# 0xk0ry/HTR-VT

Measured on NVIDIA B200. Metric: line images/sec (train step), higher is better.
Workload: dtype bf16

## Files before the change

### htr-vt_b200/csrc/attention.cu

```cuda
#include "common.cuh"
#include <cuda.h>

namespace htrvt {

constexpr int kAttnThreads = 160;
constexpr int kHd = 128;
constexpr int kTq = 128;
constexpr int kImg = kTq * 128;

__device__ __forceinline__ uint64_t desc_kmajor(uint32_t img, int k16) {
  return umma_desc_sw128(img + (k16 >> 2) * kImg + (k16 & 3) * 32, 16, 1024);
}
__device__ __forceinline__ uint64_t desc_mnmajor(uint32_t img, int k16) {
  return umma_desc_sw128(img + k16 * 2048, kImg, 1024);
}
__device__ __forceinline__ void img_store8(uint8_t* img, int r, int c, int g, uint4 v) {
  *reinterpret_cast<uint4*>(img + c * kImg + r * 128 + ((g ^ (r & 7)) << 4)) = v;
}

__device__ __forceinline__ void load_image(uint8_t* dst, const CUtensorMap* map, uint64_t* bar, int col0, int row0,
                                           int z) {
  tma_load_3d(dst, map, bar, col0, row0, z);
  tma_load_3d(dst + kImg, map, bar, col0 + 64, row0, z);
}

struct AttnP {
  int B, H, T;
  float scale;
  __nv_bfloat16* out;
  float* lse;
  const __nv_bfloat16* o;
  const __nv_bfloat16* dout;
  __nv_bfloat16* dqkv;
};

__global__ void __launch_bounds__(kAttnThreads, 2)
attn_fwd_kernel(const __grid_constant__ CUtensorMap tmQKV, const __grid_constant__ AttnP P) {
  extern __shared__ uint8_t smem_raw[];
  uint8_t* smem = reinterpret_cast<uint8_t*>((reinterpret_cast<uintptr_t>(smem_raw) + 1023) & ~uintptr_t(1023));
  uint8_t* sQ = smem;
  uint8_t* sK = smem + 2 * kImg;
  uint8_t* sV = smem + 4 * kImg;
  uint8_t* sP = sQ;
  uint64_t* bars = reinterpret_cast<uint64_t*>(smem + 6 * kImg);
  uint64_t* bar_load = bars, *bar_s = bars + 1, *bar_p = bars + 2, *bar_o = bars + 3;
  uint32_t* tmem_slot = reinterpret_cast<uint32_t*>(bars + 4);

  const int warp = threadIdx.x >> 5, lane = threadIdx.x & 31;
  const int bh = blockIdx.x, b = bh / P.H, h = bh - b * P.H;

  if (warp == 4 && lane == 0) {
    tma_prefetch_desc(&tmQKV);
    mbar_init(bar_load, 1); mbar_init(bar_s, 1); mbar_init(bar_p, 128); mbar_init(bar_o, 1);
    fence_barrier_init();
  }
  if (warp == 4) tmem_alloc(tmem_slot, 256);
  tc_fence_before();
  __syncthreads();
  tc_fence_after();
  const uint32_t tmem = *tmem_slot;
  constexpr uint32_t idesc_s = umma_idesc_bf16(128, 128, 0, 0);
  constexpr uint32_t idesc_o = umma_idesc_bf16(128, 128, 0, 1);

  if (warp == 4) {
    if (lane == 0) {
      mbar_arrive_expect_tx(bar_load, 6 * kImg);
      const int D = P.H * kHd;
      load_image(sQ, &tmQKV, bar_load, h * kHd, 0, b);
      load_image(sK, &tmQKV, bar_load, D + h * kHd, 0, b);
      load_image(sV, &tmQKV, bar_load, 2 * D + h * kHd, 0, b);
      mbar_wait(bar_load, 0);
      tc_fence_after();
      const uint32_t q = smem_u32(sQ), k = smem_u32(sK);
#pragma unroll
      for (int i = 0; i < 8; ++i) umma_bf16(tmem, desc_kmajor(q, i), desc_kmajor(k, i), idesc_s, i ? 1u : 0u);
      umma_commit(bar_s);
      mbar_wait(bar_p, 0);
      tc_fence_after();
      const uint32_t pp = smem_u32(sP), v = smem_u32(sV);
#pragma unroll
      for (int i = 0; i < 8; ++i) umma_bf16(tmem + 128, desc_kmajor(pp, i), desc_mnmajor(v, i), idesc_o, i ? 1u : 0u);
      umma_commit(bar_o);
    }
  } else {
    const int r = warp * 32 + lane;
    const uint32_t trow = tmem + (static_cast<uint32_t>(warp * 32) << 16);
    mbar_wait(bar_s, 0);
    tc_fence_after();
    float s[128];
#pragma unroll
    for (int c = 0; c < 128; c += 16) {
      uint32_t raw[16];
      tmem_ld16(trow + c, raw);
      tmem_ld_wait();
#pragma unroll
      for (int i = 0; i < 16; ++i) s[c + i] = __uint_as_float(raw[i]);
    }
    const float sl2 = P.scale * kLog2e;
    float m = -INFINITY;
#pragma unroll
    for (int j = 0; j < 128; ++j) {
      if (j >= P.T) s[j] = -INFINITY;
      m = fmaxf(m, s[j]);
    }
    float sum = 0.f;
#pragma unroll
    for (int j = 0; j < 128; ++j) {
      s[j] = ex2f((s[j] - m) * sl2);
      sum += s[j];
    }
    const float inv = __fdividef(1.0f, sum);
    asm volatile("bar.sync 1, 128;" ::: "memory");
#pragma unroll
    for (int g = 0; g < 16; ++g) {
      uint4 u;
      u.x = pack_bf16(s[8 * g], s[8 * g + 1]); u.y = pack_bf16(s[8 * g + 2], s[8 * g + 3]);
      u.z = pack_bf16(s[8 * g + 4], s[8 * g + 5]); u.w = pack_bf16(s[8 * g + 6], s[8 * g + 7]);
      img_store8(sP, r, g >> 3, g & 7, u);
    }
    fence_proxy_async();
    tc_fence_before();
    mbar_arrive(bar_p);
    if (r < P.T && P.lse) P.lse[static_cast<long long>(bh) * P.T + r] = m * P.scale + __logf(sum);
    mbar_wait(bar_o, 0);
    tc_fence_after();
    __nv_bfloat16* orow = P.out + (static_cast<long long>(b) * P.T + r) * (P.H * kHd) + h * kHd;
#pragma unroll
    for (int c = 0; c < 128; c += 16) {
      uint32_t raw[16];
      tmem_ld16(trow + 128 + c, raw);
      tmem_ld_wait();
      if (r < P.T) {
        uint4 u0, u1;
        u0.x = pack_bf16(__uint_as_float(raw[0]) * inv, __uint_as_float(raw[1]) * inv);
        u0.y = pack_bf16(__uint_as_float(raw[2]) * inv, __uint_as_float(raw[3]) * inv);
        u0.z = pack_bf16(__uint_as_float(raw[4]) * inv, __uint_as_float(raw[5]) * inv);
        u0.w = pack_bf16(__uint_as_float(raw[6]) * inv, __uint_as_float(raw[7]) * inv);
        u1.x = pack_bf16(__uint_as_float(raw[8]) * inv, __uint_as_float(raw[9]) * inv);
        u1.y = pack_bf16(__uint_as_float(raw[10]) * inv, __uint_as_float(raw[11]) * inv);
        u1.z = pack_bf16(__uint_as_float(raw[12]) * inv, __uint_as_float(raw[13]) * inv);
        u1.w = pack_bf16(__uint_as_float(raw[14]) * inv, __uint_as_float(raw[15]) * inv);
        *reinterpret_cast<uint4*>(orow + c) = u0;
        *reinterpret_cast<uint4*>(orow + c + 8) = u1;
      }
    }
  }
  tc_fence_before();
  __syncthreads();
  if (warp == 4) tmem_dealloc(tmem, 256);
}

__global__ void __launch_bounds__(kAttnThreads, 1)
attn_bwd_kernel(const __grid_constant__ CUtensorMap tmQKV, const __grid_constant__ CUtensorMap tmDO,
                const __grid_constant__ AttnP P) {
  extern __shared__ uint8_t smem_raw[];
  uint8_t* smem = reinterpret_cast<uint8_t*>((reinterpret_cast<uintptr_t>(smem_raw) + 1023) & ~uintptr_t(1023));
  uint8_t* sQ = smem;
  uint8_t* sK = smem + 2 * kImg;
  uint8_t* sV = smem + 4 * kImg;
  uint8_t* sDO = smem + 6 * kImg;
  uint8_t* sP = smem + 8 * kImg;
  uint8_t* sDS = smem + 10 * kImg;
  uint64_t* bars = reinterpret_cast<uint64_t*>(smem + 12 * kImg);
  uint64_t* bar_load = bars, *bar_s = bars + 1, *bar_p = bars + 2, *bar_g = bars + 3;
  uint32_t* tmem_slot = reinterpret_cast<uint32_t*>(bars + 4);

  const int warp = threadIdx.x >> 5, lane = threadIdx.x & 31;
  const int bh = blockIdx.x, b = bh / P.H, h = bh - b * P.H;

  if (warp == 4 && lane == 0) {
    tma_prefetch_desc(&tmQKV);
    tma_prefetch_desc(&tmDO);
    mbar_init(bar_load, 1); mbar_init(bar_s, 1); mbar_init(bar_p, 128); mbar_init(bar_g, 1);
    fence_barrier_init();
  }
  if (warp == 4) tmem_alloc(tmem_slot, 512);
  tc_fence_before();
  __syncthreads();
  tc_fence_after();
  const uint32_t tmem = *tmem_slot;
  constexpr uint32_t id_kk = umma_idesc_bf16(128, 128, 0, 0);
  constexpr uint32_t id_km = umma_idesc_bf16(128, 128, 0, 1);
  constexpr uint32_t id_mm = umma_idesc_bf16(128, 128, 1, 1);

  if (warp == 4) {
    if (lane == 0) {
      mbar_arrive_expect_tx(bar_load, 8 * kImg);
      const int Dm = P.H * kHd;
      load_image(sQ, &tmQKV, bar_load, h * kHd, 0, b);
      load_image(sK, &tmQKV, bar_load, Dm + h * kHd, 0, b);
      load_image(sV, &tmQKV, bar_load, 2 * Dm + h * kHd, 0, b);
      load_image(sDO, &tmDO, bar_load, h * kHd, 0, b);
      mbar_wait(bar_load, 0);
      tc_fence_after();
      const uint32_t q = smem_u32(sQ), k = smem_u32(sK), v = smem_u32(sV), d_o = smem_u32(sDO);
      const uint32_t pp = smem_u32(sP), ds = smem_u32(sDS);
#pragma unroll
      for (int i = 0; i < 8; ++i) umma_bf16(tmem, desc_kmajor(q, i), desc_kmajor(k, i), id_kk, i ? 1u : 0u);
#pragma unroll
      for (int i = 0; i < 8; ++i) umma_bf16(tmem + 128, desc_kmajor(d_o, i), desc_kmajor(v, i), id_kk, i ? 1u : 0u);
      umma_commit(bar_s);
      mbar_wait(bar_p, 0);
      tc_fence_after();
#pragma unroll
      for (int i = 0; i < 8; ++i) umma_bf16(tmem + 384, desc_mnmajor(pp, i), desc_mnmajor(d_o, i), id_mm, i ? 1u : 0u);
#pragma unroll
      for (int i = 0; i < 8; ++i) umma_bf16(tmem, desc_mnmajor(ds, i), desc_mnmajor(q, i), id_mm, i ? 1u : 0u);
#pragma unroll
      for (int i = 0; i < 8; ++i) umma_bf16(tmem + 256, desc_kmajor(ds, i), desc_mnmajor(k, i), id_km, i ? 1u : 0u);
      umma_commit(bar_g);
    }
  } else {
    const int r = warp * 32 + lane;
    const bool rok = r < P.T;
    const uint32_t trow = tmem + (static_cast<uint32_t>(warp * 32) << 16);
    const int D = P.H * kHd;
    float delta = 0.f;
    if (rok) {
      const uint4* po = reinterpret_cast<const uint4*>(P.o + (static_cast<long long>(b) * P.T + r) * D + h * kHd);
      const uint4* pd = reinterpret_cast<const uint4*>(P.dout + (static_cast<long long>(b) * P.T + r) * D + h * kHd);
#pragma unroll 4
      for (int i = 0; i < 16; ++i) {
        const uint4 a = __ldg(po + i), c = __ldg(pd + i);
        float2 x, y;
        x = unpack_bf16(a.x); y = unpack_bf16(c.x); delta += x.x * y.x + x.y * y.y;
        x = unpack_bf16(a.y); y = unpack_bf16(c.y); delta += x.x * y.x + x.y * y.y;
        x = unpack_bf16(a.z); y = unpack_bf16(c.z); delta += x.x * y.x + x.y * y.y;
        x = unpack_bf16(a.w); y = unpack_bf16(c.w); delta += x.x * y.x + x.y * y.y;
      }
    }
    const float lse = rok ? P.lse[static_cast<long long>(bh) * P.T + r] : 0.f;
    mbar_wait(bar_s, 0);
    tc_fence_after();
    const float sl2 = P.scale * kLog2e, lse2 = lse * kLog2e;
#pragma unroll 1
    for (int c = 0; c < 128; c += 16) {
      uint32_t rs[16], rp[16];
      tmem_ld16(trow + c, rs);
      tmem_ld16(trow + 128 + c, rp);
      tmem_ld_wait();
      float p[16], ds[16];
#pragma unroll
      for (int i = 0; i < 16; ++i) {
        const bool ok = rok && (c + i) < P.T;
        p[i] = ok ? ex2f(__uint_as_float(rs[i]) * sl2 - lse2) : 0.f;
        ds[i] = ok ? p[i] * (__uint_as_float(rp[i]) - delta) * P.scale : 0.f;
      }
#pragma unroll
      for (int g = 0; g < 2; ++g) {
        uint4 u, w;
        u.x = pack_bf16(p[8 * g], p[8 * g + 1]); u.y = pack_bf16(p[8 * g + 2], p[8 * g + 3]);
        u.z = pack_bf16(p[8 * g + 4], p[8 * g + 5]); u.w = pack_bf16(p[8 * g + 6], p[8 * g + 7]);
        w.x = pack_bf16(ds[8 * g], ds[8 * g + 1]); w.y = pack_bf16(ds[8 * g + 2], ds[8 * g + 3]);
        w.z = pack_bf16(ds[8 * g + 4], ds[8 * g + 5]); w.w = pack_bf16(ds[8 * g + 6], ds[8 * g + 7]);
        const int gg = (c >> 3) + g;
        img_store8(sP, r, gg >> 3, gg & 7, u);
        img_store8(sDS, r, gg >> 3, gg & 7, w);
      }
    }
    fence_proxy_async();
    tc_fence_before();
    mbar_arrive(bar_p);
    mbar_wait(bar_g, 0);
    tc_fence_after();
    __nv_bfloat16* base = P.dqkv + (static_cast<long long>(b) * P.T + r) * (3 * D) + h * kHd;
    const uint32_t cols[3] = {256u, 0u, 384u};
#pragma unroll 1
    for (int w = 0; w < 3; ++w) {
      __nv_bfloat16* dst = base + w * D;
#pragma unroll 1
      for (int c = 0; c < 128; c += 16) {
        uint32_t raw[16];
        tmem_ld16(trow + cols[w] + c, raw);
        tmem_ld_wait();
        if (rok) {
          uint4 u0, u1;
          u0.x = pack_bf16(__uint_as_float(raw[0]), __uint_as_float(raw[1]));
          u0.y = pack_bf16(__uint_as_float(raw[2]), __uint_as_float(raw[3]));
          u0.z = pack_bf16(__uint_as_float(raw[4]), __uint_as_float(raw[5]));
          u0.w = pack_bf16(__uint_as_float(raw[6]), __uint_as_float(raw[7]));
          u1.x = pack_bf16(__uint_as_float(raw[8]), __uint_as_float(raw[9]));
          u1.y = pack_bf16(__uint_as_float(raw[10]), __uint_as_float(raw[11]));
          u1.z = pack_bf16(__uint_as_float(raw[12]), __uint_as_float(raw[13]));
          u1.w = pack_bf16(__uint_as_float(raw[14]), __uint_as_float(raw[15]));
          *reinterpret_cast<uint4*>(dst + c) = u0;
          *reinterpret_cast<uint4*>(dst + c + 8) = u1;
        }
      }
    }
  }
  tc_fence_before();
  __syncthreads();
  if (warp == 4) tmem_dealloc(tmem, 512);
}

}

using namespace htrvt;

namespace {
typedef CUresult (*EncodeTiledFn)(CUtensorMap*, CUtensorMapDataType, cuuint32_t, void*, const cuuint64_t*,
                                  const cuuint64_t*, const cuuint32_t*, const cuuint32_t*, CUtensorMapInterleave,
                                  CUtensorMapSwizzle, CUtensorMapL2promotion, CUtensorMapFloatOOBfill);
EncodeTiledFn attn_encode() {
  static EncodeTiledFn fn = nullptr;
  if (!fn) {
    void* p = nullptr;
    cudaDriverEntryPointQueryResult q;
    if (cudaGetDriverEntryPoint("cuTensorMapEncodeTiled", &p, cudaEnableDefault, &q) == cudaSuccess &&
        q == cudaDriverEntryPointSuccess)
      fn = reinterpret_cast<EncodeTiledFn>(p);
  }
  return fn;
}
int map3(CUtensorMap* m, const void* ptr, long long cols, long long rows, long long z, long long row_stride,
         long long z_stride) {
  EncodeTiledFn enc = attn_encode();
  if (!enc) return HTRVT_ERR_DRIVER;
  if (reinterpret_cast<uintptr_t>(ptr) & 15) return HTRVT_ERR_ALIGN;
  cuuint64_t gd[3] = {static_cast<cuuint64_t>(cols), static_cast<cuuint64_t>(rows), static_cast<cuuint64_t>(z)};
  cuuint64_t gs[2] = {static_cast<cuuint64_t>(row_stride) * 2, static_cast<cuuint64_t>(z_stride) * 2};
  cuuint32_t bx[3] = {64, 128, 1}, es[3] = {1, 1, 1};
  if ((gs[0] & 15) || (gs[1] & 15)) return HTRVT_ERR_ALIGN;
  CUresult r = enc(m, CU_TENSOR_MAP_DATA_TYPE_BFLOAT16, 3, const_cast<void*>(ptr), gd, gs, bx, es,
                   CU_TENSOR_MAP_INTERLEAVE_NONE, CU_TENSOR_MAP_SWIZZLE_128B, CU_TENSOR_MAP_L2_PROMOTION_L2_256B,
                   CU_TENSOR_MAP_FLOAT_OOB_FILL_NONE);
  return r == CUDA_SUCCESS ? HTRVT_OK : HTRVT_ERR_DRIVER;
}
}

extern "C" int htrvt_attention_fwd(const void* qkv, int B, int H, int T, int hd, float scale, void* out, float* lse,
                                   cudaStream_t stream) {
  if (hd != kHd || T < 1 || T > kTq || B < 1 || H < 1) return HTRVT_ERR_SHAPE;
  CUtensorMap tm;
  int r = map3(&tm, qkv, 3LL * H * kHd, T, B, 3LL * H * kHd, static_cast<long long>(T) * 3 * H * kHd);
  if (r) return r;
  AttnP P = {};
  P.B = B; P.H = H; P.T = T; P.scale = scale; P.out = static_cast<__nv_bfloat16*>(out); P.lse = lse;
  const int smem = 6 * kImg + 1024 + 128;
  if (!HTRVT_ENSURE_SMEM(attn_fwd_kernel, smem)) return HTRVT_ERR_LAUNCH;
  attn_fwd_kernel<<<B * H, kAttnThreads, smem, stream>>>(tm, P);
  HTRVT_LAUNCH_CHECK();
  return HTRVT_OK;
}

extern "C" int htrvt_attention_bwd(const void* qkv, const void* out, const void* dout, const float* lse, int B, int H,
                                   int T, int hd, float scale, void* dqkv, cudaStream_t stream) {
  if (hd != kHd || T < 1 || T > kTq || B < 1 || H < 1 || !lse) return HTRVT_ERR_SHAPE;
  CUtensorMap tm, tdo;
  int r = map3(&tm, qkv, 3LL * H * kHd, T, B, 3LL * H * kHd, static_cast<long long>(T) * 3 * H * kHd);
  if (r) return r;
  r = map3(&tdo, dout, static_cast<long long>(H) * kHd, T, B, static_cast<long long>(H) * kHd,
           static_cast<long long>(T) * H * kHd);
  if (r) return r;
  AttnP P = {};
  P.B = B; P.H = H; P.T = T; P.scale = scale; P.lse = const_cast<float*>(lse);
  P.o = static_cast<const __nv_bfloat16*>(out); P.dout = static_cast<const __nv_bfloat16*>(dout);
  P.dqkv = static_cast<__nv_bfloat16*>(dqkv);
  const int smem = 12 * kImg + 1024 + 128;
  if (!HTRVT_ENSURE_SMEM(attn_bwd_kernel, smem)) return HTRVT_ERR_LAUNCH;
  attn_bwd_kernel<<<B * H, kAttnThreads, smem, stream>>>(tm, tdo, P);
  HTRVT_LAUNCH_CHECK();
  return HTRVT_OK;
}
```

Before: 7464.

## Make attention fwd/bwd persistent with double-buffered TMA pipeline and TMA stores

```diff
diff --git a/htr-vt_b200/csrc/attention.cu b/htr-vt_b200/csrc/attention.cu
--- a/htr-vt_b200/csrc/attention.cu
+++ b/htr-vt_b200/csrc/attention.cu
@@ -3,10 +3,14 @@
 
 namespace htrvt {
 
-constexpr int kAttnThreads = 160;
+constexpr int kRowThreads = 256;
+constexpr int kAttnThreads = kRowThreads + 64;
+constexpr int kProducerWarp = 8, kMmaWarp = 9;
 constexpr int kHd = 128;
 constexpr int kTq = 128;
 constexpr int kImg = kTq * 128;
+constexpr int kSlot = 2 * kImg;
+constexpr int kTail = 256;
 
 __device__ __forceinline__ uint64_t desc_kmajor(uint32_t img, int k16) {
   return umma_desc_sw128(img + (k16 >> 2) * kImg + (k16 & 3) * 32, 16, 1024);
@@ -16,6 +20,9 @@
 }
 __device__ __forceinline__ void img_store8(uint8_t* img, int r, int c, int g, uint4 v) {
   *reinterpret_cast<uint4*>(img + c * kImg + r * 128 + ((g ^ (r & 7)) << 4)) = v;
+}
+__device__ __forceinline__ uint4 img_load8(const uint8_t* img, int r, int c, int g) {
+  return *reinterpret_cast<const uint4*>(img + c * kImg + r * 128 + ((g ^ (r & 7)) << 4));
 }
 
 __device__ __forceinline__ void load_image(uint8_t* dst, const CUtensorMap* map, uint64_t* bar, int col0, int row0,
@@ -23,158 +30,263 @@
   tma_load_3d(dst, map, bar, col0, row0, z);
   tma_load_3d(dst + kImg, map, bar, col0 + 64, row0, z);
 }
+__device__ __forceinline__ void store_image(const CUtensorMap* map, const uint8_t* src, int col0, int row0, int z) {
+#pragma unroll
+  for (int c = 0; c < 2; ++c)
+    asm volatile("cp.async.bulk.tensor.3d.global.shared::cta.tile.bulk_group [%0, {%2, %3, %4}], [%1];"
+                 ::"l"(reinterpret_cast<uint64_t>(map)), "r"(smem_u32(src + c * kImg)), "r"(col0 + 64 * c), "r"(row0),
+                 "r"(z)
+                 : "memory");
+  asm volatile("cp.async.bulk.commit_group;" ::: "memory");
+}
+template <int N>
+__device__ __forceinline__ void bulk_wait_read() {
+  asm volatile("cp.async.bulk.wait_group.read %0;" ::"n"(N) : "memory");
+}
+__device__ __forceinline__ void bulk_wait_all() { asm volatile("cp.async.bulk.wait_group 0;" ::: "memory"); }
+__device__ __forceinline__ void row_sync() { asm volatile("barrier.sync 1, %0;" ::"n"(kRowThreads) : "memory"); }
+__device__ __forceinline__ void pair_sync(int q) { asm volatile("barrier.sync %0, 64;" ::"r"(2 + q) : "memory"); }
+
+__device__ __forceinline__ void tmem_ld64(uint32_t taddr, float (&x)[64]) {
+  uint32_t raw[4][16];
+#pragma unroll
+  for (int c = 0; c < 4; ++c) tmem_ld16(taddr + 16 * c, raw[c]);
+  tmem_ld_wait();
+#pragma unroll
+  for (int c = 0; c < 4; ++c)
+#pragma unroll
+    for (int i = 0; i < 16; ++i) x[16 * c + i] = __uint_as_float(raw[c][i]);
+}
+__device__ __forceinline__ void img_store_row64(uint8_t* img, int r, int half, const float (&x)[64], float mul) {
+#pragma unroll
+  for (int g = 0; g < 8; ++g) {
+    uint4 u;
+    u.x = pack_bf16(x[8 * g] * mul, x[8 * g + 1] * mul); u.y = pack_bf16(x[8 * g + 2] * mul, x[8 * g + 3] * mul);
+    u.z = pack_bf16(x[8 * g + 4] * mul, x[8 * g + 5] * mul); u.w = pack_bf16(x[8 * g + 6] * mul, x[8 * g + 7] * mul);
+    img_store8(img, r, half, g, u);
+  }
+}
+__device__ __forceinline__ void img_store_row64(uint8_t* img, int r, int half, const float (&x)[64]) {
+#pragma unroll
+  for (int g = 0; g < 8; ++g) {
+    uint4 u;
+    u.x = pack_bf16(x[8 * g], x[8 * g + 1]); u.y = pack_bf16(x[8 * g + 2], x[8 * g + 3]);
+    u.z = pack_bf16(x[8 * g + 4], x[8 * g + 5]); u.w = pack_bf16(x[8 * g + 6], x[8 * g + 7]);
+    img_store8(img, r, half, g, u);
+  }
+}
 
 struct AttnP {
   int B, H, T;
   float scale;
-  __nv_bfloat16* out;
   float* lse;
-  const __nv_bfloat16* o;
-  const __nv_bfloat16* dout;
-  __nv_bfloat16* dqkv;
 };
 
-__global__ void __launch_bounds__(kAttnThreads, 2)
-attn_fwd_kernel(const __grid_constant__ CUtensorMap tmQKV, const __grid_constant__ AttnP P) {
+__device__ unsigned int g_attn_sched[2][2];
+
+__device__ __forceinline__ int draw_item(unsigned int* sched, int it) {
+  return it ? static_cast<int>(gridDim.x + atomicAdd(&sched[0], 1u)) : static_cast<int>(blockIdx.x);
+}
+__device__ __forceinline__ void sched_finish(unsigned int* sched) {
+  __threadfence();
+  if (atomicAdd(&sched[1], 1u) == gridDim.x - 1) {
+    sched[0] = 0u;
+    sched[1] = 0u;
+    __threadfence();
+  }
+}
+
+constexpr int kFwdStages = 2;
+constexpr int kFwdStage = 3 * kSlot;
+constexpr int kFwdSmem = kFwdStages * kFwdStage + 1024 + kTail + 2 * 2 * kTq * 4;
+
+__global__ void __launch_bounds__(kAttnThreads, 1)
+attn_fwd_kernel(const __grid_constant__ CUtensorMap tmQKV, const __grid_constant__ CUtensorMap tmOut,
+                const __grid_constant__ AttnP P) {
   extern __shared__ uint8_t smem_raw[];
   uint8_t* smem = reinterpret_cast<uint8_t*>((reinterpret_cast<uintptr_t>(smem_raw) + 1023) & ~uintptr_t(1023));
-  uint8_t* sQ = smem;
-  uint8_t* sK = smem + 2 * kImg;
-  uint8_t* sV = smem + 4 * kImg;
-  uint8_t* sP = sQ;
-  uint64_t* bars = reinterpret_cast<uint64_t*>(smem + 6 * kImg);
-  uint64_t* bar_load = bars, *bar_s = bars + 1, *bar_p = bars + 2, *bar_o = bars + 3;
-  uint32_t* tmem_slot = reinterpret_cast<uint32_t*>(bars + 4);
+  uint8_t* tail = smem + kFwdStages * kFwdStage;
+  uint64_t* bars = reinterpret_cast<uint64_t*>(tail);
+  uint64_t* bar_full = bars;
+  uint64_t* bar_free = bars + 2;
+  uint64_t* bar_s = bars + 4;
+  uint64_t* bar_p = bars + 6;
+  uint64_t* bar_o = bars + 8;
+  uint64_t* bar_tfree = bars + 10;
+  uint32_t* tmem_slot = reinterpret_cast<uint32_t*>(bars + 12);
+  int* stage_item = reinterpret_cast<int*>(bars + 13);
+  float* xmax = reinterpret_cast<float*>(tail + kTail);
+  float* xsum = xmax + 2 * kTq;
 
   const int warp = threadIdx.x >> 5, lane = threadIdx.x & 31;
-  const int bh = blockIdx.x, b = bh / P.H, h = bh - b * P.H;
-
-  if (warp == 4 && lane == 0) {
+  const int nitems = P.B * P.H;
+
+  if (warp == kProducerWarp && lane == 0) {
     tma_prefetch_desc(&tmQKV);
-    mbar_init(bar_load, 1); mbar_init(bar_s, 1); mbar_init(bar_p, 128); mbar_init(bar_o, 1);
+    tma_prefetch_desc(&tmOut);
+    for (int s = 0; s < kFwdStages; ++s) {
+      mbar_init(&bar_full[s], 1); mbar_init(&bar_free[s], 1); mbar_init(&bar_s[s], 1);
+      mbar_init(&bar_p[s], kRowThreads); mbar_init(&bar_o[s], 1); mbar_init(&bar_tfree[s], kRowThreads);
+    }
     fence_barrier_init();
   }
-  if (warp == 4) tmem_alloc(tmem_slot, 256);
+  if (warp == kMmaWarp) tmem_alloc(tmem_slot, 512);
   tc_fence_before();
   __syncthreads();
   tc_fence_after();
   const uint32_t tmem = *tmem_slot;
   constexpr uint32_t idesc_s = umma_idesc_bf16(128, 128, 0, 0);
   constexpr uint32_t idesc_o = umma_idesc_bf16(128, 128, 0, 1);
-
-  if (warp == 4) {
+  const int D = P.H * kHd;
+
+  if (warp == kProducerWarp) {
     if (lane == 0) {
-      mbar_arrive_expect_tx(bar_load, 6 * kImg);
-      const int D = P.H * kHd;
-      load_image(sQ, &tmQKV, bar_load, h * kHd, 0, b);
-      load_image(sK, &tmQKV, bar_load, D + h * kHd, 0, b);
-      load_image(sV, &tmQKV, bar_load, 2 * D + h * kHd, 0, b);
-      mbar_wait(bar_load, 0);
+      for (int it = 0;; ++it) {
+        const int s = it & 1;
+        if (it >= kFwdStages) mbar_wait(&bar_free[s], ((it >> 1) - 1) & 1);
+        if (it >= 1) mbar_wait(&bar_full[s ^ 1], ((it - 1) >> 1) & 1);
+        const int item = draw_item(g_attn_sched[0], it);
+        if (item >= nitems) {
+          stage_item[s] = -1;
+          mbar_arrive(&bar_full[s]);
+          break;
+        }
+        stage_item[s] = item;
+        const int b = item / P.H, h = item - b * P.H;
+        uint8_t* st = smem + s * kFwdStage;
+        mbar_arrive_expect_tx(&bar_full[s], kFwdStage);
+        load_image(st, &tmQKV, &bar_full[s], h * kHd, 0, b);
+        load_image(st + kSlot, &tmQKV, &bar_full[s], D + h * kHd, 0, b);
+        load_image(st + 2 * kSlot, &tmQKV, &bar_full[s], 2 * D + h * kHd, 0, b);
+      }
+      sched_finish(g_attn_sched[0]);
+    }
+  } else if (warp == kMmaWarp) {
+    if (lane == 0) {
+      for (int it = 0;; ++it) {
+        const int s = it & 1;
+        const uint32_t ph = (it >> 1) & 1, tb = tmem + s * 256;
+        const uint32_t q = smem_u32(smem + s * kFwdStage), k = q + kSlot, v = q + 2 * kSlot;
+        mbar_wait(&bar_full[s], ph);
+        if (stage_item[s] < 0) break;
+        if (it >= kFwdStages) mbar_wait(&bar_tfree[s], ph ^ 1);
+        tc_fence_after();
+#pragma unroll
+        for (int i = 0; i < 8; ++i) umma_bf16(tb, desc_kmajor(q, i), desc_kmajor(k, i), idesc_s, i ? 1u : 0u);
+        umma_commit(&bar_s[s]);
+        mbar_wait(&bar_p[s], ph);
+        tc_fence_after();
+#pragma unroll
+        for (int i = 0; i < 8; ++i) umma_bf16(tb + 128, desc_kmajor(q, i), desc_mnmajor(v, i), idesc_o, i ? 1u : 0u);
+        umma_commit(&bar_o[s]);
+      }
+    }
+  } else {
+    const int quad = warp & 3, half = warp >> 2, r = quad * 32 + lane, c0 = half * 64;
+    const uint32_t lanes = static_cast<uint32_t>(quad * 32) << 16;
+    const float sl2 = P.scale * kLog2e;
+    for (int it = 0;; ++it) {
+      const int s = it & 1;
+      const uint32_t ph = (it >> 1) & 1, tb = tmem + s * 256 + lanes + c0;
+      mbar_wait(&bar_full[s], ph);
+      const int item = stage_item[s];
+      if (item < 0) break;
+      const int b = item / P.H, h = item - b * P.H;
+      uint8_t* sQ = smem + s * kFwdStage;
+      mbar_wait(&bar_s[s], ph);
       tc_fence_after();
-      const uint32_t q = smem_u32(sQ), k = smem_u32(sK);
-#pragma unroll
-      for (int i = 0; i < 8; ++i) umma_bf16(tmem, desc_kmajor(q, i), desc_kmajor(k, i), idesc_s, i ? 1u : 0u);
-      umma_commit(bar_s);
-      mbar_wait(bar_p, 0);
+      float x[64];
+      tmem_ld64(tb, x);
+      float m = -INFINITY;
+#pragma unroll
+      for (int j = 0; j < 64; ++j) {
+        if (c0 + j >= P.T) x[j] = -INFINITY;
+        m = fmaxf(m, x[j]);
+      }
+      xmax[half * kTq + r] = m;
+      pair_sync(quad);
+      m = fmaxf(m, xmax[(half ^ 1) * kTq + r]);
+      float sum = 0.f;
+#pragma unroll
+      for (int j = 0; j < 64; ++j) {
+        x[j] = ex2f((x[j] - m) * sl2);
+        sum += x[j];
+      }
+      xsum[half * kTq + r] = sum;
+      pair_sync(quad);
+      const float other = xsum[(half ^ 1) * kTq + r];
+      sum = half ? other + sum : sum + other;
+      const float inv = __fdividef(1.0f, sum);
+      img_store_row64(sQ, r, half, x, 1.0f);
+      fence_proxy_async();
+      tc_fence_before();
+      mbar_arrive(&bar_p[s]);
+      if (half == 0 && r < P.T && P.lse) P.lse[static_cast<long long>(item) * P.T + r] = m * P.scale + __logf(sum);
+      mbar_wait(&bar_o[s], ph);
       tc_fence_after();
-      const uint32_t pp = smem_u32(sP), v = smem_u32(sV);
-#pragma unroll
-      for (int i = 0; i < 8; ++i) umma_bf16(tmem + 128, desc_kmajor(pp, i), desc_mnmajor(v, i), idesc_o, i ? 1u : 0u);
-      umma_commit(bar_o);
-    }
-  } else {
-    const int r = warp * 32 + lane;
-    const uint32_t trow = tmem + (static_cast<uint32_t>(warp * 32) << 16);
-    mbar_wait(bar_s, 0);
-    tc_fence_after();
-    float s[128];
-#pragma unroll
-    for (int c = 0; c < 128; c += 16) {
-      uint32_t raw[16];
-      tmem_ld16(trow + c, raw);
-      tmem_ld_wait();
-#pragma unroll
-      for (int i = 0; i < 16; ++i) s[c + i] = __uint_as_float(raw[i]);
-    }
-    const float sl2 = P.scale * kLog2e;
-    float m = -INFINITY;
-#pragma unroll
-    for (int j = 0; j < 128; ++j) {
-      if (j >= P.T) s[j] = -INFINITY;
-      m = fmaxf(m, s[j]);
-    }
-    float sum = 0.f;
-#pragma unroll
-    for (int j = 0; j < 128; ++j) {
-      s[j] = ex2f((s[j] - m) * sl2);
-      sum += s[j];
-    }
-    const float inv = __fdividef(1.0f, sum);
-    asm volatile("bar.sync 1, 128;" ::: "memory");
-#pragma unroll
-    for (int g = 0; g < 16; ++g) {
-      uint4 u;
-      u.x = pack_bf16(s[8 * g], s[8 * g + 1]); u.y = pack_bf16(s[8 * g + 2], s[8 * g + 3]);
-      u.z = pack_bf16(s[8 * g + 4], s[8 * g + 5]); u.w = pack_bf16(s[8 * g + 6], s[8 * g + 7]);
-      img_store8(sP, r, g >> 3, g & 7, u);
-    }
-    fence_proxy_async();
-    tc_fence_before();
-    mbar_arrive(bar_p);
-    if (r < P.T && P.lse) P.lse[static_cast<long long>(bh) * P.T + r] = m * P.scale + __logf(sum);
-    mbar_wait(bar_o, 0);
-    tc_fence_after();
-    __nv_bfloat16* orow = P.out + (static_cast<long long>(b) * P.T + r) * (P.H * kHd) + h * kHd;
-#pragma unroll
-    for (int c = 0; c < 128; c += 16) {
-      uint32_t raw[16];
-      tmem_ld16(trow + 128 + c, raw);
-      tmem_ld_wait();
-      if (r < P.T) {
-        uint4 u0, u1;
-        u0.x = pack_bf16(__uint_as_float(raw[0]) * inv, __uint_as_float(raw[1]) * inv);
-        u0.y = pack_bf16(__uint_as_float(raw[2]) * inv, __uint_as_float(raw[3]) * inv);
-        u0.z = pack_bf16(__uint_as_float(raw[4]) * inv, __uint_as_float(raw[5]) * inv);
-        u0.w = pack_bf16(__uint_as_float(raw[6]) * inv, __uint_as_float(raw[7]) * inv);
-        u1.x = pack_bf16(__uint_as_float(raw[8]) * inv, __uint_as_float(raw[9]) * inv);
-        u1.y = pack_bf16(__uint_as_float(raw[10]) * inv, __uint_as_float(raw[11]) * inv);
-        u1.z = pack_bf16(__uint_as_float(raw[12]) * inv, __uint_as_float(raw[13]) * inv);
-        u1.w = pack_bf16(__uint_as_float(raw[14]) * inv, __uint_as_float(raw[15]) * inv);
-        *reinterpret_cast<uint4*>(orow + c) = u0;
-        *reinterpret_cast<uint4*>(orow + c + 8) = u1;
-      }
-    }
+      tmem_ld64(tb + 128, x);
+      tc_fence_before();
+      mbar_arrive(&bar_tfree[s]);
+      img_store_row64(sQ, r, half, x, inv);
+      fence_proxy_async();
+      row_sync();
+      if (threadIdx.x == 0) {
+        store_image(&tmOut, sQ, h * kHd, 0, b);
+        bulk_wait_read<0>();
+        mbar_arrive(&bar_free[s]);
+      }
+      __syncwarp();
+    }
+    if (threadIdx.x == 0) bulk_wait_all();
   }
   tc_fence_before();
   __syncthreads();
-  if (warp == 4) tmem_dealloc(tmem, 256);
-}
+  if (warp == kMmaWarp) tmem_dealloc(tmem, 512);
+}
+
+constexpr int kBwdSmem = 7 * kSlot + 1024 + kTail + 2 * kTq * 4;
 
 __global__ void __launch_bounds__(kAttnThreads, 1)
 attn_bwd_kernel(const __grid_constant__ CUtensorMap tmQKV, const __grid_constant__ CUtensorMap tmDO,
+                const __grid_constant__ CUtensorMap tmO, const __grid_constant__ CUtensorMap tmDQKV,
                 const __grid_constant__ AttnP P) {
   extern __shared__ uint8_t smem_raw[];
   uint8_t* smem = reinterpret_cast<uint8_t*>((reinterpret_cast<uintptr_t>(smem_raw) + 1023) & ~uintptr_t(1023));
   uint8_t* sQ = smem;
-  uint8_t* sK = smem + 2 * kImg;
-  uint8_t* sV = smem + 4 * kImg;
-  uint8_t* sDO = smem + 6 * kImg;
-  uint8_t* sP = smem + 8 * kImg;
-  uint8_t* sDS = smem + 10 * kImg;
-  uint64_t* bars = reinterpret_cast<uint64_t*>(smem + 12 * kImg);
-  uint64_t* bar_load = bars, *bar_s = bars + 1, *bar_p = bars + 2, *bar_g = bars + 3;
-  uint32_t* tmem_slot = reinterpret_cast<uint32_t*>(bars + 4);
+  uint8_t* sK = smem + kSlot;
+  uint8_t* sV = smem + 2 * kSlot;
+  uint8_t* sDO = smem + 3 * kSlot;
+  uint8_t* sP = smem + 4 * kSlot;
+  uint8_t* sDS = smem + 5 * kSlot;
+  uint8_t* sO = smem + 6 * kSlot;
+  uint8_t* tail = smem + 7 * kSlot;
+  uint64_t* bars = reinterpret_cast<uint64_t*>(tail);
+  uint64_t* bar_qkd = bars;
+  uint64_t* bar_v = bars + 1;
+  uint64_t* bar_ol = bars + 2;
+  uint64_t* bar_s = bars + 3;
+  uint64_t* bar_ofree = bars + 4;
+  uint64_t* bar_p = bars + 5;
+  uint64_t* bar_g = bars + 6;
+  uint64_t* bar_kfree = bars + 7;
+  uint32_t* tmem_slot = reinterpret_cast<uint32_t*>(bars + 8);
+  int* item_ring = reinterpret_cast<int*>(bars + 9);
+  float* xdel = reinterpret_cast<float*>(tail + kTail);
 
   const int warp = threadIdx.x >> 5, lane = threadIdx.x & 31;
-  const int bh = blockIdx.x, b = bh / P.H, h = bh - b * P.H;
-
-  if (warp == 4 && lane == 0) {
+  const int nitems = P.B * P.H;
+
+  if (warp == kProducerWarp && lane == 0) {
     tma_prefetch_desc(&tmQKV);
     tma_prefetch_desc(&tmDO);
-    mbar_init(bar_load, 1); mbar_init(bar_s, 1); mbar_init(bar_p, 128); mbar_init(bar_g, 1);
+    tma_prefetch_desc(&tmO);
+    tma_prefetch_desc(&tmDQKV);
+    mbar_init(bar_qkd, 1); mbar_init(bar_v, 1); mbar_init(bar_ol, 1); mbar_init(bar_s, 1);
+    mbar_init(bar_ofree, kRowThreads); mbar_init(bar_p, kRowThreads); mbar_init(bar_g, 1);
+    mbar_init(bar_kfree, kRowThreads);
     fence_barrier_init();
   }
-  if (warp == 4) tmem_alloc(tmem_slot, 512);
+  if (warp == kMmaWarp) tmem_alloc(tmem_slot, 512);
   tc_fence_before();
   __syncthreads();
   tc_fence_after();
@@ -182,116 +294,155 @@
   constexpr uint32_t id_kk = umma_idesc_bf16(128, 128, 0, 0);
   constexpr uint32_t id_km = umma_idesc_bf16(128, 128, 0, 1);
   constexpr uint32_t id_mm = umma_idesc_bf16(128, 128, 1, 1);
-
-  if (warp == 4) {
+  const int D = P.H * kHd;
+
+  if (warp == kProducerWarp) {
     if (lane == 0) {
-      mbar_arrive_expect_tx(bar_load, 8 * kImg);
-      const int Dm = P.H * kHd;
-      load_image(sQ, &tmQKV, bar_load, h * kHd, 0, b);
-      load_image(sK, &tmQKV, bar_load, Dm + h * kHd, 0, b);
-      load_image(sV, &tmQKV, bar_load, 2 * Dm + h * kHd, 0, b);
-      load_image(sDO, &tmDO, bar_load, h * kHd, 0, b);
-      mbar_wait(bar_load, 0);
-      tc_fence_after();
+      for (int it = 0;; ++it) {
+        const uint32_t prev = (it - 1) & 1;
+        if (it) mbar_wait(bar_s, prev);
+        const int item = draw_item(g_attn_sched[1], it);
+        if (item >= nitems) {
+          item_ring[it & 1] = -1;
+          mbar_arrive(bar_v);
+          if (it) mbar_wait(bar_ofree, prev);
+          mbar_arrive(bar_ol);
+          if (it) mbar_wait(bar_g, prev);
+          mbar_arrive(bar_qkd);
+          break;
+        }
+        item_ring[it & 1] = item;
+        const int b = item / P.H, h = item - b * P.H;
+        mbar_arrive_expect_tx(bar_v, kSlot);
+        load_image(sV, &tmQKV, bar_v, 2 * D + h * kHd, 0, b);
+        if (it) mbar_wait(bar_ofree, prev);
+        mbar_arrive_expect_tx(bar_ol, kSlot);
+        load_image(sO, &tmO, bar_ol, h * kHd, 0, b);
+        if (it) mbar_wait(bar_g, prev);
+        mbar_arrive_expect_tx(bar_qkd, 3 * kSlot);
+        load_image(sQ, &tmQKV, bar_qkd, h * kHd, 0, b);
+        load_image(sK, &tmQKV, bar_qkd, D + h * kHd, 0, b);
+        load_image(sDO, &tmDO, bar_qkd, h * kHd, 0, b);
+      }
+      sched_finish(g_attn_sched[1]);
+    }
+  } else if (warp == kMmaWarp) {
+    if (lane == 0) {
       const uint32_t q = smem_u32(sQ), k = smem_u32(sK), v = smem_u32(sV), d_o = smem_u32(sDO);
       const uint32_t pp = smem_u32(sP), ds = smem_u32(sDS);
-#pragma unroll
-      for (int i = 0; i < 8; ++i) umma_bf16(tmem, desc_kmajor(q, i), desc_kmajor(k, i), id_kk, i ? 1u : 0u);
-#pragma unroll
-      for (int i = 0; i < 8; ++i) umma_bf16(tmem + 128, desc_kmajor(d_o, i), desc_kmajor(v, i), id_kk, i ? 1u : 0u);
-      umma_commit(bar_s);
-      mbar_wait(bar_p, 0);
-      tc_fence_after();
-#pragma unroll
-      for (int i = 0; i < 8; ++i) umma_bf16(tmem + 384, desc_mnmajor(pp, i), desc_mnmajor(d_o, i), id_mm, i ? 1u : 0u);
-#pragma unroll
-      for (int i = 0; i < 8; ++i) umma_bf16(tmem, desc_mnmajor(ds, i), desc_mnmajor(q, i), id_mm, i ? 1u : 0u);
-#pragma unroll
-      for (int i = 0; i < 8; ++i) umma_bf16(tmem + 256, desc_kmajor(ds, i), desc_mnmajor(k, i), id_km, i ? 1u : 0u);
-      umma_commit(bar_g);
+      for (int it = 0;; ++it) {
+        const uint32_t ph = it & 1;
+        mbar_wait(bar_qkd, ph);
+        mbar_wait(bar_v, ph);
+        if (item_ring[it & 1] < 0) break;
+        if (it) mbar_wait(bar_kfree, ph ^ 1);
+        tc_fence_after();
+#pragma unroll
+        for (int i = 0; i < 8; ++i) umma_bf16(tmem, desc_kmajor(q, i), desc_kmajor(k, i), id_kk, i ? 1u : 0u);
+#pragma unroll
+        for (int i = 0; i < 8; ++i) umma_bf16(tmem + 128, desc_kmajor(d_o, i), desc_kmajor(v, i), id_kk, i ? 1u : 0u);
+        umma_commit(bar_s);
+        mbar_wait(bar_p, ph);
+        tc_fence_after();
+#pragma unroll
+        for (int i = 0; i < 8; ++i) umma_bf16(tmem + 384, desc_mnmajor(pp, i), desc_mnmajor(d_o, i), id_mm, i ? 1u : 0u);
+#pragma unroll
+        for (int i = 0; i < 8; ++i) umma_bf16(tmem, desc_mnmajor(ds, i), desc_mnmajor(q, i), id_mm, i ? 1u : 0u);
+#pragma unroll
+        for (int i = 0; i < 8; ++i) umma_bf16(tmem + 256, desc_kmajor(ds, i), desc_mnmajor(k, i), id_km, i ? 1u : 0u);
+        umma_commit(bar_g);
+      }
     }
   } else {
-    const int r = warp * 32 + lane;
+    const int quad = warp & 3, half = warp >> 2, r = quad * 32 + lane, c0 = half * 64;
     const bool rok = r < P.T;
-    const uint32_t trow = tmem + (static_cast<uint32_t>(warp * 32) << 16);
-    const int D = P.H * kHd;
-    float delta = 0.f;
-    if (rok) {
-      const uint4* po = reinterpret_cast<const uint4*>(P.o + (static_cast<long long>(b) * P.T + r) * D + h * kHd);
-      const uint4* pd = reinterpret_cast<const uint4*>(P.dout + (static_cast<long long>(b) * P.T + r) * D + h * kHd);
-#pragma unroll 4
-      for (int i = 0; i < 16; ++i) {
-        const uint4 a = __ldg(po + i), c = __ldg(pd + i);
+    const uint32_t trow = tmem + (static_cast<uint32_t>(quad * 32) << 16) + c0;
+    const float sl2 = P.scale * kLog2e;
+    for (int it = 0;; ++it) {
+      const uint32_t ph = it & 1;
+      mbar_wait(bar_ol, ph);
+      const int item = item_ring[it & 1];
+      if (item < 0) break;
+      const int b = item / P.H, h = item - b * P.H;
+      const float lse = rok ? P.lse[static_cast<long long>(item) * P.T + r] : 0.f;
+      mbar_wait(bar_qkd, ph);
+      float delta = 0.f;
+#pragma unroll
+      for (int g = 0; g < 8; ++g) {
+        const uint4 a = img_load8(sO, r, half, g), c = img_load8(sDO, r, half, g);
         float2 x, y;
         x = unpack_bf16(a.x); y = unpack_bf16(c.x); delta += x.x * y.x + x.y * y.y;
         x = unpack_bf16(a.y); y = unpack_bf16(c.y); delta += x.x * y.x + x.y * y.y;
         x = unpack_bf16(a.z); y = unpack_bf16(c.z); delta += x.x * y.x + x.y * y.y;
         x = unpack_bf16(a.w); y = unpack_bf16(c.w); delta += x.x * y.x + x.y * y.y;
       }
-    }
-    const float lse = rok ? P.lse[static_cast<long long>(bh) * P.T + r] : 0.f;
-    mbar_wait(bar_s, 0);
-    tc_fence_after();
-    const float sl2 = P.scale * kLog2e, lse2 = lse * kLog2e;
+      mbar_arrive(bar_ofree);
+      xdel[half * kTq + r] = delta;
+      pair_sync(quad);
+      const float other = xdel[(half ^ 1) * kTq + r];
+      delta = half ? other + delta : delta + other;
+      const float lse2 = lse * kLog2e;
+      mbar_wait(bar_s, ph);
+      tc_fence_after();
+      if (threadIdx.x == 0) bulk_wait_read<0>();
+      row_sync();
 #pragma unroll 1
-    for (int c = 0; c < 128; c += 16) {
-      uint32_t rs[16], rp[16];
-      tmem_ld16(trow + c, rs);
-      tmem_ld16(trow + 128 + c, rp);
-      tmem_ld_wait();
-      float p[16], ds[16];
-#pragma unroll
-      for (int i = 0; i < 16; ++i) {
-        const bool ok = rok && (c + i) < P.T;
-        p[i] = ok ? ex2f(__uint_as_float(rs[i]) * sl2 - lse2) : 0.f;
-        ds[i] = ok ? p[i] * (__uint_as_float(rp[i]) - delta) * P.scale : 0.f;
-      }
-#pragma unroll
-      for (int g = 0; g < 2; ++g) {
-        uint4 u, w;
-        u.x = pack_bf16(p[8 * g], p[8 * g + 1]); u.y = pack_bf16(p[8 * g + 2], p[8 * g + 3]);
-        u.z = pack_bf16(p[8 * g + 4], p[8 * g + 5]); u.w = pack_bf16(p[8 * g + 6], p[8 * g + 7]);
-        w.x = pack_bf16(ds[8 * g], ds[8 * g + 1]); w.y = pack_bf16(ds[8 * g + 2], ds[8 * g + 3]);
-        w.z = pack_bf16(ds[8 * g + 4], ds[8 * g + 5]); w.w = pack_bf16(ds[8 * g + 6], ds[8 * g + 7]);
-        const int gg = (c >> 3) + g;
-        img_store8(sP, r, gg >> 3, gg & 7, u);
-        img_store8(sDS, r, gg >> 3, gg & 7, w);
-      }
-    }
-    fence_proxy_async();
-    tc_fence_before();
-    mbar_arrive(bar_p);
-    mbar_wait(bar_g, 0);
-    tc_fence_after();
-    __nv_bfloat16* base = P.dqkv + (static_cast<long long>(b) * P.T + r) * (3 * D) + h * kHd;
-    const uint32_t cols[3] = {256u, 0u, 384u};
-#pragma unroll 1
-    for (int w = 0; w < 3; ++w) {
-      __nv_bfloat16* dst = base + w * D;
-#pragma unroll 1
-      for (int c = 0; c < 128; c += 16) {
-        uint32_t raw[16];
-        tmem_ld16(trow + cols[w] + c, raw);
+      for (int c = 0; c < 64; c += 16) {
+        uint32_t rs[16], rp[16];
+        tmem_ld16(trow + c, rs);
+        tmem_ld16(trow + 128 + c, rp);
         tmem_ld_wait();
-        if (rok) {
-          uint4 u0, u1;
-          u0.x = pack_bf16(__uint_as_float(raw[0]), __uint_as_float(raw[1]));
-          u0.y = pack_bf16(__uint_as_float(raw[2]), __uint_as_float(raw[3]));
-          u0.z = pack_bf16(__uint_as_float(raw[4]), __uint_as_float(raw[5]));
-          u0.w = pack_bf16(__uint_as_float(raw[6]), __uint_as_float(raw[7]));
-          u1.x = pack_bf16(__uint_as_float(raw[8]), __uint_as_float(raw[9]));
-          u1.y = pack_bf16(__uint_as_float(raw[10]), __uint_as_float(raw[11]));
-          u1.z = pack_bf16(__uint_as_float(raw[12]), __uint_as_float(raw[13]));
-          u1.w = pack_bf16(__uint_as_float(raw[14]), __uint_as_float(raw[15]));
-          *reinterpret_cast<uint4*>(dst + c) = u0;
-          *reinterpret_cast<uint4*>(dst + c + 8) = u1;
+        float p[16], ds[16];
+#pragma unroll
+        for (int i = 0; i < 16; ++i) {
+          const bool ok = rok && (c0 + c + i) < P.T;
+          p[i] = ok ? ex2f(__uint_as_float(rs[i]) * sl2 - lse2) : 0.f;
+          ds[i] = ok ? p[i] * (__uint_as_float(rp[i]) - delta) * P.scale : 0.f;
         }
-      }
-    }
+#pragma unroll
+        for (int g = 0; g < 2; ++g) {
+          uint4 u, w;
+          u.x = pack_bf16(p[8 * g], p[8 * g + 1]); u.y = pack_bf16(p[8 * g + 2], p[8 * g + 3]);
+          u.z = pack_bf16(p[8 * g + 4], p[8 * g + 5]); u.w = pack_bf16(p[8 * g + 6], p[8 * g + 7]);
+          w.x = pack_bf16(ds[8 * g], ds[8 * g + 1]); w.y = pack_bf16(ds[8 * g + 2], ds[8 * g + 3]);
+          w.z = pack_bf16(ds[8 * g + 4], ds[8 * g + 5]); w.w = pack_bf16(ds[8 * g + 6], ds[8 * g + 7]);
+          img_store8(sP, r, half, (c >> 3) + g, u);
+          img_store8(sDS, r, half, (c >> 3) + g, w);
+        }
+      }
+      fence_proxy_async();
+      tc_fence_before();
+      mbar_arrive(bar_p);
+      mbar_wait(bar_g, ph);
+      tc_fence_after();
+      float x[64];
+      tmem_ld64(trow, x);
+      tc_fence_before();
+      mbar_arrive(bar_kfree);
+      img_store_row64(sP, r, half, x);
+      tmem_ld64(trow + 256, x);
+      img_store_row64(sDS, r, half, x);
+      fence_proxy_async();
+      row_sync();
+      if (threadIdx.x == 0) {
+        store_image(&tmDQKV, sP, D + h * kHd, 0, b);
+        store_image(&tmDQKV, sDS, h * kHd, 0, b);
+        bulk_wait_read<1>();
+      }
+      __syncwarp();
+      tmem_ld64(trow + 384, x);
+      row_sync();
+      img_store_row64(sP, r, half, x);
+      fence_proxy_async();
+      row_sync();
+      if (threadIdx.x == 0) store_image(&tmDQKV, sP, 2 * D + h * kHd, 0, b);
+      __syncwarp();
+    }
+    if (threadIdx.x == 0) bulk_wait_all();
   }
   tc_fence_before();
   __syncthreads();
-  if (warp == 4) tmem_dealloc(tmem, 512);
+  if (warp == kMmaWarp) tmem_dealloc(tmem, 512);
 }
 
 }
@@ -327,19 +478,40 @@
                    CU_TENSOR_MAP_FLOAT_OOB_FILL_NONE);
   return r == CUDA_SUCCESS ? HTRVT_OK : HTRVT_ERR_DRIVER;
 }
+int map_btc(CUtensorMap* m, const void* ptr, long long cols, int T, int B) {
+  return map3(m, ptr, cols, T, B, cols, static_cast<long long>(T) * cols);
+}
+template <typename Kernel>
+int persistent_grid(Kernel kern, int smem, int items) {
+  static int slots[64] = {0};
+  int dev = 0;
+  cudaGetDevice(&dev);
+  dev &= 63;
+  if (!slots[dev]) {
+    int sms = 0, per_sm = 0;
+    if (cudaDeviceGetAttribute(&sms, cudaDevAttrMultiProcessorCount, dev) != cudaSuccess ||
+        cudaOccupancyMaxActiveBlocksPerMultiprocessor(&per_sm, kern, kAttnThreads, smem) != cudaSuccess)
+      return 0;
+    slots[dev] = sms * per_sm;
+  }
+  return slots[dev] < items ? slots[dev] : items;
+}
 }
 
 extern "C" int htrvt_attention_fwd(const void* qkv, int B, int H, int T, int hd, float scale, void* out, float* lse,
                                    cudaStream_t stream) {
   if (hd != kHd || T < 1 || T > kTq || B < 1 || H < 1) return HTRVT_ERR_SHAPE;
-  CUtensorMap tm;
-  int r = map3(&tm, qkv, 3LL * H * kHd, T, B, 3LL * H * kHd, static_cast<long long>(T) * 3 * H * kHd);
+  CUtensorMap tm, to;
+  int r = map_btc(&tm, qkv, 3LL * H * kHd, T, B);
+  if (r) return r;
+  r = map_btc(&to, out, static_cast<long long>(H) * kHd, T, B);
   if (r) return r;
   AttnP P = {};
-  P.B = B; P.H = H; P.T = T; P.scale = scale; P.out = static_cast<__nv_bfloat16*>(out); P.lse = lse;
-  const int smem = 6 * kImg + 1024 + 128;
-  if (!HTRVT_ENSURE_SMEM(attn_fwd_kernel, smem)) return HTRVT_ERR_LAUNCH;
-  attn_fwd_kernel<<<B * H, kAttnThreads, smem, stream>>>(tm, P);
+  P.B = B; P.H = H; P.T = T; P.scale = scale; P.lse = lse;
+  if (!HTRVT_ENSURE_SMEM(attn_fwd_kernel, kFwdSmem)) return HTRVT_ERR_LAUNCH;
+  const int grid = persistent_grid(attn_fwd_kernel, kFwdSmem, B * H);
+  if (grid < 1) return HTRVT_ERR_LAUNCH;
+  attn_fwd_kernel<<<grid, kAttnThreads, kFwdSmem, stream>>>(tm, to, P);
   HTRVT_LAUNCH_CHECK();
   return HTRVT_OK;
 }
@@ -347,19 +519,18 @@
 extern "C" int htrvt_attention_bwd(const void* qkv, const void* out, const void* dout, const float* lse, int B, int H,
                                    int T, int hd, float scale, void* dqkv, cudaStream_t stream) {
   if (hd != kHd || T < 1 || T > kTq || B < 1 || H < 1 || !lse) return HTRVT_ERR_SHAPE;
-  CUtensorMap tm, tdo;
-  int r = map3(&tm, qkv, 3LL * H * kHd, T, B, 3LL * H * kHd, static_cast<long long>(T) * 3 * H * kHd);
-  if (r) return r;
-  r = map3(&tdo, dout, static_cast<long long>(H) * kHd, T, B, static_cast<long long>(H) * kHd,
-           static_cast<long long>(T) * H * kHd);
+  CUtensorMap tm, tdo, to, tdq;
+  int r = map_btc(&tm, qkv, 3LL * H * kHd, T, B);
+  if (!r) r = map_btc(&tdo, dout, static_cast<long long>(H) * kHd, T, B);
+  if (!r) r = map_btc(&to, out, static_cast<long long>(H) * kHd, T, B);
+  if (!r) r = map_btc(&tdq, dqkv, 3LL * H * kHd, T, B);
   if (r) return r;
   AttnP P = {};
   P.B = B; P.H = H; P.T = T; P.scale = scale; P.lse = const_cast<float*>(lse);
-  P.o = static_cast<const __nv_bfloat16*>(out); P.dout = static_cast<const __nv_bfloat16*>(dout);
-  P.dqkv = static_cast<__nv_bfloat16*>(dqkv);
-  const int smem = 12 * kImg + 1024 + 128;
-  if (!HTRVT_ENSURE_SMEM(attn_bwd_kernel, smem)) return HTRVT_ERR_LAUNCH;
-  attn_bwd_kernel<<<B * H, kAttnThreads, smem, stream>>>(tm, tdo, P);
+  if (!HTRVT_ENSURE_SMEM(attn_bwd_kernel, kBwdSmem)) return HTRVT_ERR_LAUNCH;
+  const int grid = persistent_grid(attn_bwd_kernel, kBwdSmem, B * H);
+  if (grid < 1) return HTRVT_ERR_LAUNCH;
+  attn_bwd_kernel<<<grid, kAttnThreads, kBwdSmem, stream>>>(tm, tdo, to, tdq, P);
   HTRVT_LAUNCH_CHECK();
   return HTRVT_OK;
 }
```

New measurement: 7533 (median of 6 runs). About the same (+0.9%).
